# trioxane/consensus_clustering

Hardware: AMD Instinct MI355X
Metric: consensus fit wall-time + resample-clusterings/sec, n=50k d=128, 1/2/4/8 GPU (higher is better)
Workload: dtype f16x3 hi/lo, f32 accumulate (k-means MFMA) / i8 (co-association MFMA)

## Files before the change

consensus_clustering_amd/csrc/kmeans.hip:

```cpp
#include <hip/hip_runtime.h>

#include <algorithm>
#include <climits>
#include <cmath>
#include <cstdlib>
#include <cstdint>
#include <string>
#include <vector>

#include "kmeans_shared.hpp"

namespace {

using namespace cc::km;

constexpr int NT = 512;
constexpr int NW = 8;
constexpr int NDW = 4;
constexpr int NEW = NW - NDW;
constexpr int RT = 32;
constexpr int CW = 256;
constexpr int NLS = 8;
constexpr int NSS = 8;
constexpr int NLS_D = 3;
// ... 56 lines not shown
  const float* xnorm;
  int dreal;
  float scale, inv_scale, dscale, ndinv;
  const int32_t* idx;
  int m, h_begin, nh, T;
  const int32_t* units;
  int nU;
  int max_iter;
  double tol_rel;
  const double* kpp_u;
  int kpp_stride, n_init;
  const int32_t* kpp_pos;
  uint8_t* labels_out;
  int n, ldl, H;
  float* inertia_out;
  int32_t* niter_out;
  unsigned long long* stats;
  unsigned* counter;
  uint8_t* ws;
  size_t ws_per_wg, off_cen, off_cenn, off_cpos, off_dbuf, off_rdist, off_s64, off_c64, off_list;
  int Pws, Kws, Tws, seedmax;
  int lsm;
  int lseg;
};

__device__ int cc_km_dense_only = 0;
__device__ int cc_km_share_seed = 1;

struct State {
  int unit, P;
  float tol;
  int rr;
  unsigned seedfree;
  unsigned char K[PMAX], kidx[PMAX], init[PMAX], ntr[PMAX], st[PMAX], c[PMAX], cs[PMAX], sslot[PMAX];
  unsigned char need_sel[PMAX], to_run[PMAX], sbest[PMAX], lcur[PMAX];
  short cenoff[PMAX], pitem[PMAX];
  int iter[PMAX], amax[PMAX], nempty[PMAX];
  int pchg[PMAX];
  float pot32[PMAX], inert[PMAX];
  int cand[PMAX][TMAX];
  int nitems, ncols;
  unsigned char ikind[IMAX], iprob[IMAX], itr[IMAX];
  unsigned iw0[IMAX], iw1[IMAX];
  unsigned char lstep[NW][NLS], sstep[NW][NSS][2];
  unsigned char nlw[NW], nsw[NW];
  int4 sdesc[NW][NSS][2];
// ... 171 lines not shown
      const float t = x[d] - c[d];
      s = fmaf(t, t, s);
    }
    dist[r] = s;
    mymax = fmaxf(mymax, s);
  }
  for (int o = 32; o > 0; o >>= 1) mymax = fmaxf(mymax, __shfl_xor(mymax, o));
  if ((tid & 63) == 0) S.red_v[tid >> 6] = mymax;
  __syncthreads();
  double gmax = 0.0;
  for (int w = 0; w < NW; ++w) gmax = fmax(gmax, S.red_v[w]);
  if (tid == 0) {
    int ne = 0;
    for (int c = 0; c < K; ++c)
      if (S.cnt[off + c] == 0) S.map[ne++] = c;
    S.flag = ne;
  }
  __syncthreads();
  if (gmax == 0.0) return;
  relocate_farthest<NT, NW>(m, S.flag, S.map, dist, glab, a.X, idx, DP, off, Sm, S.cnt, S.red_v, S.red_i,
                            S.n_reloc, tid);
}

__device__ unsigned list_changes(const uint8_t* cur, const uint8_t* old, int m, int w, int lane, uint2* seg,
                                 unsigned cap) {
  const int rs = (((m + NW - 1) / NW) + 15) & ~15;
  const int r0 = w * rs, r1 = min(m, r0 + rs);
  unsigned n = 0;
  for (int b = r0; b < r1; b += 16 * 64) {
    const int r = b + 16 * lane;
    unsigned msk = 0;
    uint4 x = make_uint4(0, 0, 0, 0), y = x;
    if (r < r1) {
      x = *reinterpret_cast<const uint4*>(cur + r);
      y = *reinterpret_cast<const uint4*>(old + r);
      const unsigned xs[4] = {x.x, x.y, x.z, x.w}, ys[4] = {y.x, y.y, y.z, y.w};
#pragma unroll
      for (int q = 0; q < 4; ++q) {
        const unsigned dq = xs[q] ^ ys[q];
#pragma unroll
        for (int k = 0; k < 4; ++k) msk |= ((dq >> (8 * k)) & 0xFFu) ? (1u << (4 * q + k)) : 0u;
      }
    }
    const unsigned c = __popc(msk);
    unsigned pre = c;
#pragma unroll
    for (int o = 1; o < 64; o <<= 1) {
      const unsigned t = __shfl_up(pre, o);
      if (lane >= o) pre += t;
    }
    unsigned pos = n + pre - c;
    const unsigned xs[4] = {x.x, x.y, x.z, x.w}, ys[4] = {y.x, y.y, y.z, y.w};
    while (msk) {
      const int k = __builtin_ctz(msk);
      msk &= msk - 1;
      const unsigned nv = (xs[k >> 2] >> (8 * (k & 3))) & 0xFFu, ov = (ys[k >> 2] >> (8 * (k & 3))) & 0xFFu;
      if (pos < cap) seg[pos] = make_uint2(static_cast<unsigned>(r + k), ov | (nv << 8));
      ++pos;
    }
    n += __shfl(pre, 63);
  }
  return n;
}

template <int DP>
__device__ void apply_changes(const KArgs& a, const int32_t* idx, const uint2* lst, const unsigned* nseg,
                              bool full, const uint8_t* lab, float* acc, unsigned* cnt, int K, int lane) {
  constexpr int DL = DP >= 64 ? DP / 64 : 1;
  const bool dok = lane * DL < DP;
  const int d0 = dok ? lane * DL : 0;
  for (int e = lane; e < K * DP; e += 64) acc[e] = 0.f;
  if (lane < K) cnt[lane] = 0u;
  for (int sg = 0; sg < (full ? 1 : NW); ++sg) {
    const int n = full ? a.m : static_cast<int>(nseg[sg]);
    const uint2* ls = lst + static_cast<size_t>(sg) * a.lseg;
    for (int e0 = 0; e0 < n; e0 += 64) {
      const int e = e0 + lane;
      unsigned xr = 0, o = 0xFFu, nw = 0xFFu;
      if (e < n) {
        unsigned r;
        if (full) {
          r = static_cast<unsigned>(e);
          nw = lab[e];
// ... 39 lines not shown
                *reinterpret_cast<float2*>(q) = t;
              } else {
                *q += v[j][0];
              }
            }
            if (jo[j] < 0xFFu) {
              float* q = acc + jo[j] * DP + d0;
              if constexpr (DL == 2) {
                float2 t = *reinterpret_cast<float2*>(q);
                t.x -= v[j][0];
                t.y -= v[j][DL - 1];
                *reinterpret_cast<float2*>(q) = t;
              } else {
                *q -= v[j][0];
              }
            }
          }
        }
      }
    }
  }
}

typedef float v4f __attribute__((ext_vector_type(4)));
typedef float v2f __attribute__((ext_vector_type(2)));
typedef double v2d __attribute__((ext_vector_type(2)));
#define KM_GLOBAL __attribute__((address_space(1)))
#define KM_LDS __attribute__((address_space(3)))
template <class T>
__device__ __forceinline__ T* as_lds(T* p) {
  return (T*)(KM_LDS T*)p;
}

template <int DP>
struct SlotHalf {
  static constexpr int NQ = DP / 8;
  bool run = false;
  int p = 0, cl = 0, rot = 0;
  KM_LDS v4f* row = nullptr;
  template <class St>
  __device__ __forceinline__ SlotHalf(float* Sm, const St& S, int ncols) {
    const int tid = threadIdx.x, sl = tid >> 1;
    rot = tid / (128 / DP);
    row = (KM_LDS v4f*)(KM_LDS float*)Sm + (sl * DP + (tid & 1) * (DP / 2)) / 4;
    if (sl < ncols) {
      const int it = S.sitem[sl];
      if (it >= 0 && S.ikind[it] == IK_RUN) {
        run = true;
        p = S.iprob[it];
        cl = sl - S.ioff[it];
      }
    }
  }
  __device__ __forceinline__ int q(int j) const { return (j + rot) & (NQ - 1); }
};
// ... 64 lines not shown
      act[u] = true;
      rowu[u] = S.cenoff[S.iprob[it]] + (sl - S.ioff[it]);
      if (!(S.ichanged[it] & 2u)) {
        v[u] = s64[rowu[u] * (DP / 2) + lane];
        cu[u] = c64[rowu[u]];
      }
    }
#pragma unroll
    for (int u = 0; u < U; ++u) {
      if (!act[u]) continue;
      const int sl = s0 + u;
      const v2f f = Sm[sl * (DP / 2) + lane];
      const v2d t = {v[u].x + static_cast<double>(f.x), v[u].y + static_cast<double>(f.y)};
      s64[rowu[u] * (DP / 2) + lane] = t;
      Sm[sl * (DP / 2) + lane] = v2f{static_cast<float>(t.x), static_cast<float>(t.y)};
      if (lane == 0) {
        const int c = cu[u] + static_cast<int>(S.cnt[sl]);
        c64[rowu[u]] = c;
        S.cnt[sl] = static_cast<unsigned>(c);
      }
    }
  }
}
#undef KM_GLOBAL
#undef KM_LDS

template <class St>
__device__ void kpp_select(const KArgs& a, St& S, int p, const float* closest, int lane) {
  const int ntr = S.ntr[p];
  cc::km::kpp_select<RT, TMAX>(closest, a.m, a.T, kpp_uniforms(a.kpp_u, S.kidx[p], a.n_init, S.init[p], a.kpp_stride, S.c[p], ntr),
                               ntr, static_cast<double>(S.pot32[p]), S.cand[p], lane);
}

template <int NL, int NS>
struct EState {
  float iaccL[NL], iaccS[NS];
};
constexpr int FLUSH = 32;

__host__ __device__ constexpr int mstep_tile(int q) { return (q + 1) % NDW; }
static_assert(NEW == NDW, "one E/M wave per distance wave");

__device__ __forceinline__ int4 seed_desc(const KArgs& a, const State& S, int it, int T1) {
  if (it == 0xFF) return make_int4(0, CW, 0, CW);
  const unsigned w0 = S.iw0[it], w1 = S.iw1[it];
  const int slot = w1 & 31;
  const int dcf = iw_off(w0) | ((1 | ((iw_kind(w0) == IK_SEED) ? 2 : 0)) << 16);
  return make_int4((slot * T1 + ((w1 >> 8) & 7)) * a.lsm, dcf, (slot * T1 + ((w1 >> 11) & 7)) * a.lsm, dcf);
// ... 287 lines not shown
        }
      sacc0[dt] = mfma16(oh0, bh, sacc0[dt]);
      __builtin_amdgcn_sched_barrier(0);
#pragma unroll
      for (int k = 0; k < 4; ++k) rc[k] = rn[k];
    }
  }
}

template <int DP>
__device__ __forceinline__ void msum_out(const KArgs& a, State& S, float* Sm, const v16f (&sacc)[DP / 32],
                                         unsigned mcnt, int ct, int msl, int lr, int hh) {
#pragma unroll
  for (int dt = 0; dt < DP / 32; ++dt)
#pragma unroll
    for (int v = 0; v < 16; ++v) {
      const int s2 = 32 * ct + (v & 3) + 8 * (v >> 2) + 4 * hh;
      Sm[s2 * DP + 32 * dt + lr] = sacc[dt][v] * a.inv_scale;
    }
  const unsigned tot = mcnt + __shfl_xor(mcnt, 32);
  if (hh == 0) S.cnt[msl] = tot;
}

__device__ void schedule(const KArgs& a, State& S, const int32_t* idx, int dist_cost, bool sparse_ok) {
  const int P = S.P;
  for (int p = 0; p < P && S.seedfree; ++p) {
    if (S.st[p] != ST_WAIT) continue;
    const int s = __ffs(S.seedfree) - 1;
    S.seedfree &= ~(1u << s);
    S.sslot[p] = static_cast<unsigned char>(s);
    S.st[p] = ST_SEED;
    S.c[p] = 0;
  }
  int ni = 0, nc = 0, nls = 0, nss2 = 0;
  unsigned long long nseed = 0, nlloyd = 0, nm = 0;
  for (int p = 0; p < P; ++p) S.pitem[p] = -1;
  for (int p = 0; p < P; ++p) {
    if (S.st[p] != ST_SEED) continue;
    const int c = S.c[p];
    const int nt = (c == 0) ? 1 : S.ntr[p];
    if (nc + nt > CW || ni + nt > IMAX || nss2 + nt > 2 * (NEW * NSS + NDW * NSS_D)) continue;
    nss2 += nt;
    S.pitem[p] = static_cast<short>(ni);
    for (int t = 0; t < nt; ++t) {
      const int kind = (c == 0) ? IK_SEED0 : IK_SEED;
      S.ikind[ni] = static_cast<unsigned char>(kind);
      S.iprob[ni] = static_cast<unsigned char>(p);
// ... 91 lines not shown
    if (S.ikind[it] >= IK_RUN) continue;
    if (open_w >= 0) {
      S.sstep[open_w][S.nsw[open_w] - 1][1] = static_cast<unsigned char>(it);
      open_w = -1;
      continue;
    }
    int w = -1;
    for (int q = 0; q < NW; ++q)
      if (S.nsw[q] < (q < NDW ? NSS_D : NSS) && (w < 0 || wcost[q] < wcost[w])) w = q;
    S.sstep[w][S.nsw[w]++][0] = static_cast<unsigned char>(it);
    wcost[w] += KM_COST_SSTEP;
    open_w = w;
  }
  S.nitems = ni;
  S.ncols = nc;
  S.n_seed += nseed;
  S.n_lloyd += nlloyd;
  S.n_mrows += nm;
  if (ni > 0) {
    S.n_sweeps += 1;
    S.n_ctiles += static_cast<unsigned long long>((nc + 31) / 32) * a.T;
  }
}

template <int DP>
__global__ __launch_bounds__(NT, 1) void kmeans_kernel(KArgs a) {
  using LY = Lay<DP>;
  __shared__ __attribute__((aligned(16))) char smem[LY::TOTAL];
  char* ring = smem;
  float* Dt = reinterpret_cast<float*>(smem + LY::OFF_D);
  float* Sm = reinterpret_cast<float*>(smem);
  uint8_t* Ls = reinterpret_cast<uint8_t*>(smem + LY::OFF_LS);
  float* XN = reinterpret_cast<float*>(smem + LY::OFF_XN);
  State& S = *reinterpret_cast<State*>(smem + LY::OFF_ST);

  const int tid = threadIdx.x, lane = tid & 63;
  const int wave = __builtin_amdgcn_readfirstlane(tid >> 6);
  const int m = a.m, T = a.T;
  uint8_t* wsb = a.ws + static_cast<size_t>(blockIdx.x) * a.ws_per_wg;
  uint8_t* glab = wsb;
  double* s64 = reinterpret_cast<double*>(wsb + a.off_s64);
  int* c64 = reinterpret_cast<int*>(wsb + a.off_c64);
  uint2* clist = reinterpret_cast<uint2*>(wsb + a.off_list);
  float* cen = reinterpret_cast<float*>(wsb + a.off_cen);
  float* cenn = reinterpret_cast<float*>(wsb + a.off_cenn);
  int32_t* cpos = reinterpret_cast<int32_t*>(wsb + a.off_cpos);
  float* dbuf = reinterpret_cast<float*>(wsb + a.off_dbuf);
  float* rdist = reinterpret_cast<float*>(wsb + a.off_rdist);
  const int T1 = a.Tws + 1;
  if (tid == 0) S.n_lloyd = S.n_seed = S.n_mrows = S.n_reloc = S.n_sweeps = S.n_ctiles = S.n_sparse = S.n_changes = 0;

  for (;;) {
    __syncthreads();
    if (tid == 0) S.unit = static_cast<int>(atomicAdd(a.counter, 1u));
    __syncthreads();
    const int unit = S.unit;
    if (unit >= a.nh * a.nU) break;
    const int hb = unit / a.nU, g = unit - hb * a.nU;
    const int h = a.h_begin + hb;
    const int32_t* idx = a.idx + static_cast<size_t>(h) * m;
    const int32_t* gd = a.units + g * US;

    if (tid == 0) {
      const int P = gd[0];
      S.P = P;
      int o = 0;
      for (int p = 0; p < P; ++p) {
        S.K[p] = static_cast<unsigned char>(gd[1 + 4 * p]);
        S.kidx[p] = static_cast<unsigned char>(gd[2 + 4 * p]);
        S.init[p] = static_cast<unsigned char>(gd[3 + 4 * p]);
        S.ntr[p] = static_cast<unsigned char>(gd[4 + 4 * p]);
        S.st[p] = ST_WAIT;
        S.iter[p] = 0;
        S.pchg[p] = a.m;
        S.lcur[p] = 0;
        S.cenoff[p] = static_cast<short>(o);
        o += S.K[p];
        S.lead[p] = static_cast<unsigned char>(p);
        S.fgo[p] = 0;
      }
      if (cc_km_share_seed)
        for (int p = 0; p < P; ++p) {
          if (S.init[p] != 0) continue;
          int l = p;
          for (int q = 0; q < P; ++q)
            if (S.init[q] == 0 && S.ntr[q] == S.ntr[p] && (S.K[q] > S.K[l] || (S.K[q] == S.K[l] && q < l))) l = q;
          if (l != p) {
            S.lead[p] = static_cast<unsigned char>(l);
            S.st[p] = ST_FOLLOW;
          }
        }
      S.rr = 0;
      S.seedfree = (a.seedmax >= 32) ? 0xFFFFFFFFu : ((1u << a.seedmax) - 1u);
    }
    __syncthreads();
    const int P = S.P;
    for (size_t e = tid; e < static_cast<size_t>(2 * P) * a.lsm; e += NT) glab[e] = 0xFF;

    {
      double* red = reinterpret_cast<double*>(ring);
      double* mean = reinterpret_cast<double*>(ring) + NT;
      constexpr int NPH = NT / DP;
      const int d = tid % DP, ph = tid / DP;
      double s = 0.0;
      for (int r = ph; r < m; r += NPH) s += static_cast<double>(a.X[static_cast<size_t>(idx[r]) * DP + d]);
      red[ph * DP + d] = s;
      __syncthreads();
      if (tid < DP) {
        double t = 0.0;
        for (int k = 0; k < NPH; ++k) t += red[k * DP + tid];
        mean[tid] = t / m;
      }
      __syncthreads();
      const double mu = mean[d];
      double q = 0.0;
      for (int r = ph; r < m; r += NPH) {
        const double v = static_cast<double>(a.X[static_cast<size_t>(idx[r]) * DP + d]) - mu;
        q += v * v;
      }
      __syncthreads();
      red[ph * DP + d] = q;
      __syncthreads();
      if (tid == 0) {
        double tot = 0.0;
        for (int dd = 0; dd < a.dreal; ++dd) {
          double t = 0.0;
          for (int k = 0; k < NPH; ++k) t += red[k * DP + dd];
          tot += t / m;
        }
        S.tol = static_cast<float>(static_cast<float>(tot / a.dreal) * a.tol_rel);
      }
      __syncthreads();
    }

    for (;;) {
      KM_STAMP(swp);
      if (tid == 0) {
        if constexpr (kPair<DP>) {
          [[clang::always_inline]] schedule(a, S, idx, dist_cost<DP>(), kSparse<DP> && !cc_km_dense_only);
        } else {
          schedule(a, S, idx, dist_cost<DP>(), kSparse<DP> && !cc_km_dense_only);
        }
      }
      __syncthreads();
      const int nitems = S.nitems, ncols = S.ncols;
      if (nitems == 0) break;

      if (tid < ncols) {
        const int sr = S.srow[tid];
        S.cnorm[tid] = (sr >= 0) ? a.xnorm[sr] : (sr == INT_MIN ? __builtin_huge_valf() : cenn[-sr - 1]);
      }
      if (tid < 2 * RT * 4) Dt[(tid >> 2) * DSD + CW + (tid & 3)] = __builtin_huge_valf();
      if (tid < IMAX) S.iinert[tid] = 0.0;
      if (tid < NW * NSS * 2) {
        const int w = tid / (2 * NSS), i = (tid / 2) % NSS, h = tid & 1;
        S.sdesc[w][i][h] = seed_desc(a, S, S.sstep[w][i][h], T1);
      }
      const int hh = lane >> 5, lr = lane & 31;
      const bool pm = kPair<DP> && ncols <= 4 * 32;
      const int TP = (T + 1) >> 1;
#ifdef CC_KM_STAMPS
      unsigned long long st_acc[8] = {0, 0, 0, 0, 0, 0, 0, 0};
#endif
      if (wave < NDW) {
        const int nsub = __builtin_amdgcn_readfirstlane(static_cast<int>(32 * wave < ncols) +
                                                        static_cast<int>(32 * (wave + NDW) < ncols));
        h8 ah0[DP / 16], al0[DP / 16], ah1[DP / 16], al1[DP / 16];
// ... 235 lines not shown
        for (int k = 0; k < 7; ++k) atomicAdd(&a.stats[8 + 8 * wave + k], st_acc[k]);
#endif
      __syncthreads();

      KM_STAMP(pp0);
      if (tid < P) {
        const int p = tid;
        S.need_sel[p] = 0;
        S.to_run[p] = S.fgo[p];
        if (S.st[p] == ST_SEED && S.pitem[p] >= 0) {
          const int c = S.c[p];
          const KppDecision k = kpp_decide(S.iinert + S.pitem[p], S.ntr[p], c, S.cs[p]);
          S.pot32[p] = k.pot;
          S.cs[p] = static_cast<unsigned char>(k.cs);
          S.sbest[p] = static_cast<unsigned char>(k.best);
          cpos[p * a.Kws + c] = (c == 0) ? a.kpp_pos[S.kidx[p] * a.n_init + S.init[p]] : S.cand[p][k.best];
          S.c[p] = static_cast<unsigned char>(c + 1);
          if (c + 1 == S.K[p]) {
            S.to_run[p] = 1;
          } else {
            S.need_sel[p] = 1;
          }
        }
      }
      __syncthreads();
      if (tid == 0) {
        for (int p = 0; p < P; ++p)
          if (S.to_run[p]) {
            if (S.st[p] == ST_SEED) S.seedfree |= 1u << S.sslot[p];
            S.st[p] = ST_RUN;
            S.iter[p] = 0;
            S.pchg[p] = a.m;
          }
      }
      {
        int j = 0;
        for (int p = 0; p < P; ++p) {
          if (!S.need_sel[p]) continue;
          if ((j++ % NW) != wave) continue;
          const int ss = S.sslot[p];
          if constexpr (kPair<DP>) {
            [[clang::always_inline]] kpp_select(a, S, p, dbuf + (static_cast<size_t>(ss) * T1 + S.cs[p]) * a.lsm, lane);
          } else {
            kpp_select(a, S, p, dbuf + (static_cast<size_t>(ss) * T1 + S.cs[p]) * a.lsm, lane);
          }
        }
      }
      for (int p = 0; p < P; ++p) {
        if (!S.to_run[p]) continue;
        const int K = S.K[p], cp = S.lead[p] * a.Kws;
        for (int e = tid; e < K * DP; e += NT) {
          const int c = e / DP, d = e - c * DP;
          cen[(S.cenoff[p] + c) * DP + d] = a.X[static_cast<size_t>(idx[cpos[cp + c]]) * DP + d];
        }
        if (tid < K) cenn[S.cenoff[p] + tid] = row_sq(a.X + static_cast<size_t>(idx[cpos[cp + tid]]) * DP, a.dreal);
      }

// ... 18 lines not shown
            for (int w = 0; w < NW; ++w) {
              tot += S.lcnt[it][w];
              over |= S.lcnt[it][w] > static_cast<unsigned>(a.lseg);
            }
            S.pchg[S.iprob[it]] = static_cast<int>(tot);
            S.ichanged[it] = (tot != 0) | ((S.isparse[it] && over) ? 2u : 0u);
#ifdef CC_KM_STAMPS
            if (S.isparse[it] && over && a.stats) atomicAdd(&a.stats[117], 1ull);
#endif
          }
        }
      } else {
        if (tid < nitems) S.ichanged[tid] = 0;
        __syncthreads();
        for (int it = 0; it < nitems; ++it) {
          if (S.ikind[it] != IK_RUN) continue;
          const int p = S.iprob[it];
          if (labels_differ<NT>(glab + static_cast<size_t>(2 * p + 1 - S.lcur[p]) * a.lsm,
                                glab + static_cast<size_t>(2 * p + S.lcur[p]) * a.lsm, m, tid))
            S.ichanged[it] = 1;
        }
      }
      __syncthreads();
      if (tid == 0)
        for (int it = 0; it < nitems; ++it)
          if (S.ikind[it] >= IK_RUN) {
            S.lcur[S.iprob[it]] = static_cast<unsigned char>(1 - S.lcur[S.iprob[it]]);
            if (S.ikind[it] == IK_RUN) S.n_changes += static_cast<unsigned>(S.pchg[S.iprob[it]]);
          }
      __syncthreads();
      KM_STAMP(ppB);

      if constexpr (kSparse<DP>) {
        for (int e = tid; e < ncols * DP; e += NT) {
          const int sl = e / DP, d = e - sl * DP;
          const int it = S.sitem[sl];
          if (it < 0 || S.ikind[it] != IK_RUN || S.isparse[it] || sl - S.ioff[it] >= S.K[S.iprob[it]]) continue;
          const int row = S.cenoff[S.iprob[it]] + (sl - S.ioff[it]);
          s64[static_cast<size_t>(row) * DP + d] = static_cast<double>(Sm[e]);
          if (d == 0) c64[row] = static_cast<int>(S.cnt[sl]);
        }
        KM_STAMP(rs0);
        {
          int j = 0;
          for (int it = 0; it < nitems; ++it) {
            if (S.ikind[it] != IK_RUN || !S.isparse[it]) continue;
            if ((j++ % NW) != wave) continue;
            const int p = S.iprob[it], off = S.ioff[it];
            apply_changes<DP>(a, idx, clist + static_cast<size_t>(p) * NW * a.lseg, S.lcnt[it], (S.ichanged[it] & 2u) != 0,
                              glab + static_cast<size_t>(2 * p + S.lcur[p]) * a.lsm, Sm + static_cast<size_t>(off) * DP,
                              S.cnt + off, S.K[p], lane);
          }
        }
        KM_STAMP(rs1);
        __syncthreads();
        KM_STAMP(rs2);
        add_sparse_deltas<DP>(Sm, S, s64, c64, ncols);
        KM_STAMP(rs3);
        __syncthreads();
#ifdef CC_KM_STAMPS
        if (blockIdx.x == 0 && tid == 0 && a.stats) {
          atomicAdd(&a.stats[112], rs0 - ppB);
          atomicAdd(&a.stats[113], rs1 - rs0);
          atomicAdd(&a.stats[114], rs3 - rs2);
          atomicAdd(&a.stats[115], rs2 - rs1);
        }
#endif
      }

      KM_STAMP(ppC);
      if (tid == 0) {
        int f = 0;
        for (int it = 0; it < nitems; ++it) {
          if (S.ikind[it] != IK_RUN) continue;
          const int p = S.iprob[it], off = S.ioff[it];
          int ne = 0;
          for (int c = 0; c < S.K[p]; ++c) ne += (S.cnt[off + c] == 0);
          S.nempty[p] = ne;
          f |= (ne > 0);
        }
        S.flag = f;
      }
      __syncthreads();
      if (S.flag) {
        for (int it = 0; it < nitems; ++it) {
          if (S.ikind[it] != IK_RUN) continue;
          const int p = S.iprob[it];
          if (S.nempty[p] == 0) continue;
          if constexpr (kPair<DP>) {
            [[clang::always_inline]] relocate<DP>(a, idx, p, S.ioff[it], cen, Sm, S,
                                                  glab + static_cast<size_t>(2 * p + S.lcur[p]) * a.lsm, rdist, tid);
          } else {
            relocate<DP>(a, idx, p, S.ioff[it], cen, Sm, S, glab + static_cast<size_t>(2 * p + S.lcur[p]) * a.lsm,
                         rdist, tid);
          }
          __syncthreads();
        }
      }
      if (tid < nitems && S.ikind[tid] == IK_RUN) {
        const int p = S.iprob[tid], off = S.ioff[tid];
        int am = 0;
        for (int c = 1; c < S.K[p]; ++c)
          if (S.cnt[off + c] > S.cnt[off + am]) am = c;
        S.amax[p] = am;
      }
      __syncthreads();
// ... 29 lines not shown
                                        a.max_iter, S.iter[p]);
        S.st[p] = static_cast<unsigned char>(st);
        if (st == ST_DONE) S.inert[p] = static_cast<float>(S.iinert[it]);
      }
      __syncthreads();
      write_centres<DP>(Sm, S, cen, ncols);
      if (tid < ncols) {
        const int it = S.sitem[tid];
        if (it >= 0 && S.ikind[it] == IK_RUN) {
          const int p = S.iprob[it];
          if (S.st[p] != ST_DONE) cenn[S.cenoff[p] + (tid - S.ioff[it])] = row_sq(Sm + tid * DP, a.dreal);
        }
      }
      __syncthreads();
#ifdef CC_KM_STAMPS
      KM_STAMP(pp1);
      if (blockIdx.x == 0 && tid == 0 && a.stats) {
        atomicAdd(&a.stats[73], pp1 - pp0);
        atomicAdd(&a.stats[106], ppA - pp0);
        atomicAdd(&a.stats[107], ppB - ppA);
        atomicAdd(&a.stats[108], ppC - ppB);
        atomicAdd(&a.stats[109], pp1 - ppC);
        atomicAdd(&a.stats[116], cu1 - cu0);
      }
      if (tid == 0 && a.stats) {
        const int wv = (ncols + 31) / 32;
        atomicAdd(&a.stats[80 + wv], pp1 - swp);
        atomicAdd(&a.stats[96 + wv], 1ull);
        if (S.ikind[0] < IK_RUN) {
          atomicAdd(&a.stats[110], pp1 - swp);
          atomicAdd(&a.stats[111], 1ull);
        }
      }
#endif
    }

    for (int p0 = 0; p0 < P; p0 += a.n_init) {
      const auto lab = [&](int p) { return glab + static_cast<size_t>(2 * p + S.lcur[p]) * a.lsm; };
      const int best = best_of_inits<NT, KMAX>(p0, a.n_init, m, lab, [&](int p) { return S.inert[p]; }, S.map, S.flag, tid);
      write_fit<NT>(lab(best), idx, m, a.labels_out, a.n, a.ldl, S.kidx[p0], h, a.H, S.inert[best], S.iter[best],
                    a.inertia_out, a.niter_out, tid);
    }
  }
  if (tid == 0 && a.stats) {
    atomicAdd(&a.stats[0], S.n_lloyd);
    atomicAdd(&a.stats[1], S.n_seed);
    atomicAdd(&a.stats[2], S.n_mrows);
    atomicAdd(&a.stats[3], S.n_reloc);
    atomicAdd(&a.stats[4], S.n_sweeps);
    atomicAdd(&a.stats[5], S.n_ctiles);
    atomicAdd(&a.stats[6], S.n_sparse);
    atomicAdd(&a.stats[7], S.n_changes);
  }
}

__global__ void split_kernel(const float* X, long long total, int dpad, float scale, uint16_t* Xhl) {
  const long long i = static_cast<long long>(blockIdx.x) * blockDim.x + threadIdx.x;
  if (i >= total) return;
  const long long row = i / dpad;
  const int d = static_cast<int>(i - row * dpad);
  const float xs = X[i] * scale;
  const _Float16 hi = static_cast<_Float16>(xs);
  const _Float16 lo = static_cast<_Float16>(xs - static_cast<float>(hi));
  Xhl[row * 2 * dpad + d] = __builtin_bit_cast(uint16_t, hi);
  Xhl[row * 2 * dpad + dpad + d] = __builtin_bit_cast(uint16_t, lo);
}

struct WsLayout {
  int Pws = 0, Cws = 0, Kws = 0, Tws = 0, lseg = 0;
  size_t off_cen = 0, off_cenn = 0, off_cpos = 0, off_dbuf = 0, off_rdist = 0, off_s64 = 0, off_c64 = 0,
         off_list = 0, per_wg = 0;
};

int list_seg(int m) { return std::max(16, ((m / 16) + 15) & ~15); }

constexpr size_t WS_HEADER = 256;

WsLayout ws_layout(int m, int dpad, const int32_t* units, int nU, int seedmax) {
  WsLayout L;
  for (int g = 0; g < nU; ++g) {
    const int32_t* gd = units + static_cast<size_t>(g) * US;
    L.Pws = std::max(L.Pws, gd[0]);
    int cols = 0;
    for (int p = 0; p < gd[0]; ++p) {
      L.Kws = std::max(L.Kws, gd[1 + 4 * p]);
      L.Tws = std::max(L.Tws, gd[4 + 4 * p]);
      cols += gd[1 + 4 * p];
    }
    L.Cws = std::max(L.Cws, cols);
  }
  const auto al = align256;
  L.off_cen = al(static_cast<size_t>(2 * L.Pws) * ((m + 63) & ~63));
  L.off_cenn = L.off_cen + al(static_cast<size_t>(L.Cws) * dpad * sizeof(float));
  L.off_cpos = L.off_cenn + al(static_cast<size_t>(L.Cws) * sizeof(float));
  L.off_dbuf = L.off_cpos + al(static_cast<size_t>(L.Pws) * L.Kws * sizeof(int32_t));
  L.off_rdist = L.off_dbuf + al(static_cast<size_t>(seedmax) * (L.Tws + 1) * ((m + 63) & ~63) * sizeof(float));
  const bool sp = dpad == 128;
  L.off_s64 = L.off_rdist + al(static_cast<size_t>(m) * sizeof(float));
  L.off_c64 = L.off_s64 + (sp ? al(static_cast<size_t>(L.Cws) * dpad * sizeof(double)) : 0);
  L.off_list = L.off_c64 + (sp ? al(static_cast<size_t>(L.Cws) * sizeof(int)) : 0);
  L.lseg = list_seg(m);
  L.per_wg = L.off_list + (sp ? al(static_cast<size_t>(L.Pws) * NW * L.lseg * sizeof(uint2)) : 0);
  return L;
}

template <int DP>
void launch(const KArgs& a, unsigned blocks, hipStream_t st) {
  hipLaunchKernelGGL(kmeans_kernel<DP>, dim3(blocks), dim3(NT), 0, st, a);
}

}

extern "C" int cc_kmeans_plan(const int32_t* Ks, int nK, int n_init, int n_sub, int32_t* units,
                              int max_units) {
  if (!Ks || nK <= 0 || n_init <= 0 || n_sub <= 0 || !units || max_units <= 0) {
    cc::set_error("cc_kmeans_plan: bad arguments");
    return CC_ERR_ARG;
  }
  if (n_init > PMAX) {
    cc::set_error("cc_kmeans_plan: n_init must be <= 64");
    return CC_ERR_UNSUPPORTED;
  }
  std::vector<int> order(nK);
  for (int i = 0; i < nK; ++i) {
    if (Ks[i] < 1 || Ks[i] > KMAX) {
// ... 141 lines not shown
  a.kpp_u = kpp_u;
  a.kpp_stride = kpp_stride;
  a.n_init = n_init;
  a.kpp_pos = kpp_pos;
  a.labels_out = labels_nh;
  a.n = n;
  a.ldl = ldl;
  a.H = H;
  a.inertia_out = inertia;
  a.niter_out = n_iter;
  a.stats = stats;
  a.counter = static_cast<unsigned*>(workspace);
  a.ws = static_cast<uint8_t*>(workspace) + WS_HEADER;
  a.ws_per_wg = L.per_wg;
  a.off_cen = L.off_cen;
  a.off_cenn = L.off_cenn;
  a.off_cpos = L.off_cpos;
  a.off_dbuf = L.off_dbuf;
  a.off_rdist = L.off_rdist;
  a.off_s64 = L.off_s64;
  a.off_c64 = L.off_c64;
  a.off_list = L.off_list;
  a.lseg = L.lseg;
  a.Pws = L.Pws;
  a.Kws = L.Kws;
  a.Tws = L.Tws;
  a.seedmax = seedmax;
  a.lsm = (m + 63) & ~63;
  {
    static int dense_set = 0;
    const char* dm = std::getenv("CCMI_KM_DENSE");
    const int dense = (dm && dm[0] == '1') ? 1 : 0;
    if (dense != dense_set) {
      e = hipMemcpyToSymbolAsync(HIP_SYMBOL(cc_km_dense_only), &dense, sizeof(int), 0, hipMemcpyHostToDevice, st);
      if (e != hipSuccess) return hip_fail("cc_kmeans_batched", e);
      dense_set = dense;
    }
    static int share_set = 1;
    const char* sm = std::getenv("CCMI_KM_SHARE_SEED");
    const int share = (sm && sm[0] == '0') ? 0 : 1;
    if (share != share_set) {
      e = hipMemcpyToSymbolAsync(HIP_SYMBOL(cc_km_share_seed), &share, sizeof(int), 0, hipMemcpyHostToDevice, st);
      if (e != hipSuccess) return hip_fail("cc_kmeans_batched", e);
      share_set = share;
    }
    if (const char* ls = std::getenv("CCMI_KM_LSEG")) {
// ... 13 lines not shown
```

Measured before the change: 11330.

## Parallelize k-means scheduler across a wave and unroll serial per-sweep loops

Result: faster. 11850, median of 6 (+4.6%).

```diff
diff --git a/consensus_clustering_amd/csrc/kmeans.hip b/consensus_clustering_amd/csrc/kmeans.hip
--- a/consensus_clustering_amd/csrc/kmeans.hip
+++ b/consensus_clustering_amd/csrc/kmeans.hip
@@ -102,6 +102,9 @@
   int Pws, Kws, Tws, seedmax;
   int lsm;
   int lseg;
+#ifdef CC_KM_SCHED_CHECK
+  size_t off_chk;
+#endif
 };
 
 __device__ int cc_km_dense_only = 0;
@@ -319,43 +322,83 @@
                             S.n_reloc, tid);
 }
 
-__device__ unsigned list_changes(const uint8_t* cur, const uint8_t* old, int m, int w, int lane, uint2* seg,
-                                 unsigned cap) {
+typedef float v4f __attribute__((ext_vector_type(4)));
+typedef float v2f __attribute__((ext_vector_type(2)));
+typedef double v2d __attribute__((ext_vector_type(2)));
+typedef unsigned v4u __attribute__((ext_vector_type(4)));
+typedef unsigned v2u __attribute__((ext_vector_type(2)));
+#define KM_GLOBAL __attribute__((address_space(1)))
+#define KM_LDS __attribute__((address_space(3)))
+template <class T>
+__device__ __forceinline__ T* as_lds(T* p) {
+  return (T*)(KM_LDS T*)p;
+}
+template <class T>
+__device__ __forceinline__ KM_GLOBAL T* as_global(T* p) {
+  return (KM_GLOBAL T*)reinterpret_cast<uintptr_t>(p);
+}
+
+#ifndef KM_CMP_NB
+#define KM_CMP_NB 6
+#endif
+__device__ __noinline__ unsigned list_changes(const uint8_t* cur_, const uint8_t* old_, int m, int w, int lane,
+                                              uint2* seg_, unsigned cap) {
+  const KM_GLOBAL uint8_t* cur = as_global(cur_);
+  const KM_GLOBAL uint8_t* old = as_global(old_);
+  KM_GLOBAL v2u* seg = (KM_GLOBAL v2u*)reinterpret_cast<uintptr_t>(seg_);
+  constexpr int NB = KM_CMP_NB, BR = 16 * 64;
   const int rs = (((m + NW - 1) / NW) + 15) & ~15;
   const int r0 = w * rs, r1 = min(m, r0 + rs);
-  unsigned n = 0;
-  for (int b = r0; b < r1; b += 16 * 64) {
-    const int r = b + 16 * lane;
-    unsigned msk = 0;
-    uint4 x = make_uint4(0, 0, 0, 0), y = x;
-    if (r < r1) {
-      x = *reinterpret_cast<const uint4*>(cur + r);
-      y = *reinterpret_cast<const uint4*>(old + r);
-      const unsigned xs[4] = {x.x, x.y, x.z, x.w}, ys[4] = {y.x, y.y, y.z, y.w};
+  unsigned n = 0, cl = 0;
+  for (int b0 = r0; b0 < r1; b0 += NB * BR) {
+    v4u x[NB], y[NB];
+#pragma unroll
+    for (int u = 0; u < NB; ++u) {
+      const int r = b0 + u * BR + 16 * lane;
+      x[u] = y[u] = v4u{0u, 0u, 0u, 0u};
+      if (r < r1) {
+        x[u] = *reinterpret_cast<const KM_GLOBAL v4u*>(cur + r);
+        y[u] = *reinterpret_cast<const KM_GLOBAL v4u*>(old + r);
+      }
+    }
+#pragma unroll
+    for (int u = 0; u < NB; ++u) {
+      if (b0 + u * BR >= r1) break;
+      const int r = b0 + u * BR + 16 * lane;
+      unsigned msk = 0;
 #pragma unroll
       for (int q = 0; q < 4; ++q) {
-        const unsigned dq = xs[q] ^ ys[q];
+        const unsigned dq = x[u][q] ^ y[u][q];
 #pragma unroll
         for (int k = 0; k < 4; ++k) msk |= ((dq >> (8 * k)) & 0xFFu) ? (1u << (4 * q + k)) : 0u;
       }
-    }
-    const unsigned c = __popc(msk);
-    unsigned pre = c;
-#pragma unroll
-    for (int o = 1; o < 64; o <<= 1) {
-      const unsigned t = __shfl_up(pre, o);
-      if (lane >= o) pre += t;
-    }
-    unsigned pos = n + pre - c;
-    const unsigned xs[4] = {x.x, x.y, x.z, x.w}, ys[4] = {y.x, y.y, y.z, y.w};
-    while (msk) {
-      const int k = __builtin_ctz(msk);
-      msk &= msk - 1;
-      const unsigned nv = (xs[k >> 2] >> (8 * (k & 3))) & 0xFFu, ov = (ys[k >> 2] >> (8 * (k & 3))) & 0xFFu;
-      if (pos < cap) seg[pos] = make_uint2(static_cast<unsigned>(r + k), ov | (nv << 8));
-      ++pos;
-    }
-    n += __shfl(pre, 63);
+      const unsigned c = __popc(msk);
+      if (cap == 0u) {
+        cl += c;
+        continue;
+      }
+      if (__ballot(msk != 0u) == 0ull) continue;
+      unsigned pre = c;
+#pragma unroll
+      for (int o = 1; o < 64; o <<= 1) {
+        const unsigned t = __shfl_up(pre, o);
+        if (lane >= o) pre += t;
+      }
+      unsigned pos = n + pre - c;
+      while (msk) {
+        const int k = __builtin_ctz(msk);
+        msk &= msk - 1;
+        const unsigned nv = (x[u][k >> 2] >> (8 * (k & 3))) & 0xFFu, ov = (y[u][k >> 2] >> (8 * (k & 3))) & 0xFFu;
+        if (pos < cap) seg[pos] = v2u{static_cast<unsigned>(r + k), ov | (nv << 8)};
+        ++pos;
+      }
+      n += __shfl(pre, 63);
+    }
+  }
+  if (cap == 0u) {
+#pragma unroll
+    for (int o = 32; o > 0; o >>= 1) cl += __shfl_xor(cl, o);
+    n = cl;
   }
   return n;
 }
@@ -441,15 +484,6 @@
   }
 }
 
-typedef float v4f __attribute__((ext_vector_type(4)));
-typedef float v2f __attribute__((ext_vector_type(2)));
-typedef double v2d __attribute__((ext_vector_type(2)));
-#define KM_GLOBAL __attribute__((address_space(1)))
-#define KM_LDS __attribute__((address_space(3)))
-template <class T>
-__device__ __forceinline__ T* as_lds(T* p) {
-  return (T*)(KM_LDS T*)p;
-}
 
 template <int DP>
 struct SlotHalf {
@@ -560,8 +594,6 @@
     }
   }
 }
-#undef KM_GLOBAL
-#undef KM_LDS
 
 template <class St>
 __device__ void kpp_select(const KArgs& a, St& S, int p, const float* closest, int lane) {
@@ -895,7 +927,8 @@
   if (hh == 0) S.cnt[msl] = tot;
 }
 
-__device__ void schedule(const KArgs& a, State& S, const int32_t* idx, int dist_cost, bool sparse_ok) {
+#ifdef CC_KM_SCHED_CHECK
+__device__ __noinline__ void schedule(const KArgs& a, State& S, const int32_t* idx, int dist_cost, bool sparse_ok) {
   const int P = S.P;
   for (int p = 0; p < P && S.seedfree; ++p) {
     if (S.st[p] != ST_WAIT) continue;
@@ -1033,6 +1066,259 @@
     S.n_ctiles += static_cast<unsigned long long>((nc + 31) / 32) * a.T;
   }
 }
+#endif
+
+#ifndef KM_TOL_U
+#define KM_TOL_U 16
+#endif
+template <int DP, bool SQ>
+__device__ __noinline__ double tol_pass(const float* X_, const int32_t* idx_, int m, double mu) {
+  const KM_GLOBAL float* X = as_global(X_);
+  const KM_GLOBAL int32_t* idx = as_global(idx_);
+  constexpr int NPH = NT / DP, U = KM_TOL_U;
+  const int d = threadIdx.x % DP, ph = threadIdx.x / DP;
+  const auto add = [&](double s, float x) {
+    if constexpr (SQ) {
+      const double v = static_cast<double>(x) - mu;
+      return __builtin_fma(v, v, s);
+    } else {
+      return s + static_cast<double>(x);
+    }
+  };
+  double s = 0.0;
+  int r = ph;
+  for (; r + (U - 1) * NPH < m; r += U * NPH) {
+    int ix[U];
+    float x[U];
+#pragma unroll
+    for (int u = 0; u < U; ++u) ix[u] = idx[r + u * NPH];
+#pragma unroll
+    for (int u = 0; u < U; ++u) x[u] = X[static_cast<size_t>(ix[u]) * DP + d];
+#pragma unroll
+    for (int u = 0; u < U; ++u) s = add(s, x[u]);
+  }
+  for (; r < m; r += NPH) s = add(s, X[static_cast<size_t>(idx[r]) * DP + d]);
+  return s;
+}
+
+__device__ __forceinline__ int lpt_wave(const int (&wcost)[NW], const int (&nst)[NW], int cap_d, int cap_e) {
+  int w = -1, best = 0;
+#pragma unroll
+  for (int q = 0; q < NW; ++q)
+    if (nst[q] < (q < NDW ? cap_d : cap_e) && (w < 0 || wcost[q] < best)) {
+      w = q;
+      best = wcost[q];
+    }
+  return w;
+}
+
+__device__ void schedule_wave(State& S_, const int32_t* idx_, const int32_t* kpp_pos_, int n_init, int m, int T,
+                              int dist_cost, bool sparse_ok, int lane) {
+  State& S = *as_lds(&S_);
+  const KM_GLOBAL int32_t* idx = as_global(idx_);
+  const KM_GLOBAL int32_t* kpp_pos = as_global(kpp_pos_);
+  const int P = __builtin_amdgcn_readfirstlane(S.P);
+  const bool in = lane < P;
+  int st = in ? S.st[lane] : 0xFF;
+  int c = in ? S.c[lane] : 0;
+  const int K = in ? S.K[lane] : 0, ntr = in ? S.ntr[lane] : 0;
+  const int lead = in ? S.lead[lane] : 0;
+  const int pchg = in ? S.pchg[lane] : 0;
+  {
+    unsigned seedfree = __builtin_amdgcn_readfirstlane(S.seedfree);
+    unsigned long long wait = __ballot(st == ST_WAIT);
+    int s_new = -1;
+    while (wait && seedfree) {
+      const int p = __builtin_ctzll(wait), s = __builtin_ctz(seedfree);
+      wait &= wait - 1;
+      seedfree &= seedfree - 1;
+      if (lane == p) s_new = s;
+    }
+    if (s_new >= 0) {
+      st = ST_SEED;
+      c = 0;
+      S.sslot[lane] = static_cast<unsigned char>(s_new);
+      S.st[lane] = ST_SEED;
+      S.c[lane] = 0;
+    }
+    if (lane == 0) S.seedfree = seedfree;
+  }
+  int ni = 0, nc = 0, nss2 = 0;
+  int myit = -1;
+  const int ntv = (c == 0) ? 1 : ntr;
+  for (unsigned long long sm = __ballot(st == ST_SEED); sm; sm &= sm - 1) {
+    const int p = __builtin_ctzll(sm);
+    const int nt = __builtin_amdgcn_readlane(ntv, p);
+    if (nc + nt > CW || ni + nt > IMAX || nss2 + nt > 2 * (NEW * NSS + NDW * NSS_D)) continue;
+    nss2 += nt;
+    if (lane == p) myit = ni;
+    ni += nt;
+    nc += nt;
+  }
+  const int nis = ni;
+  if (st == ST_SEED && myit >= 0) {
+    const int kind = (c == 0) ? IK_SEED0 : IK_SEED;
+    const int cs = (kind == IK_SEED0) ? 0 : S.cs[lane];
+    const unsigned sslot = S.sslot[lane];
+    for (int t = 0; t < ntv; ++t) {
+      const int it = myit + t;
+      S.ikind[it] = static_cast<unsigned char>(kind);
+      S.iprob[it] = static_cast<unsigned char>(lane);
+      S.ioff[it] = static_cast<short>(it);
+      S.incol[it] = 1;
+      S.itr[it] = static_cast<unsigned char>(t);
+      const int wslot = (kind == IK_SEED0) ? 0 : ((t < cs) ? t : t + 1);
+      S.iw0[it] = (static_cast<unsigned>(kind) << 24) | (static_cast<unsigned>(lane) << 16) | (1u << 8) |
+                  static_cast<unsigned>(it);
+      S.iw1[it] = (static_cast<unsigned>(wslot) << 11) | (static_cast<unsigned>(cs) << 8) |
+                  (static_cast<unsigned>(t) << 5) | sslot;
+      const int pos = (c == 0) ? kpp_pos[S.kidx[lane] * n_init + S.init[lane]] : S.cand[lane][t];
+      S.sitem[it] = static_cast<short>(it);
+      S.scl[it] = -1;
+      S.srow[it] = idx[pos];
+    }
+  }
+  {
+    const int stl = __shfl(st, lead), itl = __shfl(myit, lead), cl = __shfl(c, lead);
+    if (in) S.fgo[lane] = static_cast<unsigned char>(st == ST_FOLLOW && stl == ST_SEED && itl >= 0 && cl + 1 == K);
+  }
+  const bool lrun = st == ST_RUN || st == ST_FINAL;
+  const int sparse = (sparse_ok && st == ST_RUN && pchg <= m / 8) ? 1 : 0;
+  const int K4 = (K + 3) & ~3;
+  int nls = 0, first_skip = -1, last = -1, nrun = 0, nsp = 0, klloyd = 0;
+  int myoff = 0, itK = 0;
+  const int rr = __builtin_amdgcn_readfirstlane(S.rr);
+  {
+    const unsigned long long rm = __ballot(lrun), below = rr ? (~0ull >> (64 - rr)) : 0ull;
+#pragma unroll 1
+    for (int half = 0; half < 2; ++half)
+      for (unsigned long long q = half ? (rm & below) : (rm & ~below); q; q &= q - 1) {
+        const int p = __builtin_ctzll(q);
+        const int Kp = __builtin_amdgcn_readlane(K, p), K4p = __builtin_amdgcn_readlane(K4, p);
+        const int off = (nc + 3) & ~3;
+        if (off + K4p > CW || ni + 1 > IMAX || nls + 1 > NEW * NLS + NDW * NLS_D) {
+          if (first_skip < 0) first_skip = p;
+          continue;
+        }
+        if (lane == p) {
+          myit = ni;
+          myoff = off;
+        }
+        if (lane == nls) itK = Kp;
+        ++ni;
+        ++nls;
+        nc = off + K4p;
+        last = p;
+        klloyd += Kp;
+        nrun += __builtin_amdgcn_readlane(static_cast<int>(st == ST_RUN), p);
+        nsp += __builtin_amdgcn_readlane(sparse, p);
+      }
+  }
+  const bool litem = lrun && myit >= nis;
+  if (litem) {
+    if (myit == nis)
+      for (int s = nis; s < myoff; ++s) {
+        S.sitem[s] = -1;
+        S.scl[s] = -1;
+        S.srow[s] = INT_MIN;
+      }
+    const int kind = (st == ST_RUN) ? IK_RUN : IK_FINAL;
+    S.isparse[myit] = static_cast<unsigned char>(sparse);
+    S.ikind[myit] = static_cast<unsigned char>(kind);
+    S.iprob[myit] = static_cast<unsigned char>(lane);
+    S.ioff[myit] = static_cast<short>(myoff);
+    S.incol[myit] = static_cast<short>(K);
+    S.itr[myit] = 0;
+    S.iw0[myit] = (static_cast<unsigned>(1 - S.lcur[lane]) << 30) | (static_cast<unsigned>(kind) << 24) |
+                  (static_cast<unsigned>(lane) << 16) | (static_cast<unsigned>(K) << 8) | static_cast<unsigned>(myoff);
+    S.iw1[myit] = 0;
+    const int cenoff = S.cenoff[lane];
+    const bool msl = st == ST_RUN && !sparse;
+    for (int s = 0; s < K4; ++s) {
+      S.sitem[myoff + s] = static_cast<short>(s < K ? myit : -1);
+      S.scl[myoff + s] = static_cast<short>((msl && s < K) ? s : -1);
+      S.srow[myoff + s] = (s < K) ? -(cenoff + s) - 1 : INT_MIN;
+    }
+  }
+  if (in) S.pitem[lane] = static_cast<short>(myit);
+  int wcost[NW], nlw[NW], nsw[NW];
+  {
+    const bool dense = litem && st == ST_RUN && !sparse;
+    unsigned mt = 0;
+#pragma unroll
+    for (int j = 0; j < CW / 32; ++j)
+      if (__ballot(dense && (myoff >> 5) <= j && j <= ((myoff + K - 1) >> 5)) != 0ull) mt |= 1u << j;
+#pragma unroll
+    for (int w = 0; w < NW; ++w) {
+      wcost[w] = 0;
+      nlw[w] = nsw[w] = 0;
+      if (w < NDW) {
+#pragma unroll
+        for (int j = w; j < CW / 32; j += NDW) wcost[w] += (32 * j < nc) ? dist_cost : 0;
+      } else {
+#pragma unroll
+        for (int j = mstep_tile(w - NDW); j < CW / 32; j += NEW) wcost[w] += ((mt >> j) & 1u) ? KM_COST_MSTEP : 0;
+      }
+    }
+  }
+  static_assert(NW * NLS == 64 && NW * NSS * 2 == 128, "the step tables are reset a lane each");
+  (&S.lstep[0][0])[lane] = 0xFF;
+  (&S.sstep[0][0][0])[2 * lane] = 0xFF;
+  (&S.sstep[0][0][0])[2 * lane + 1] = 0xFF;
+  for (int i = 0; i < nls; ++i) {
+    const int Ki = __builtin_amdgcn_readlane(itK, i);
+    const int w = lpt_wave(wcost, nlw, NLS_D, NLS);
+    int n = 0;
+#pragma unroll
+    for (int q = 0; q < NW; ++q)
+      if (q == w) {
+        n = nlw[q]++;
+        wcost[q] += (Ki + 7) / 8 * KM_COST_LCHUNK + KM_COST_LBASE;
+      }
+    if (lane == 0) S.lstep[w][n] = static_cast<unsigned char>(nis + i);
+  }
+  for (int it = 0; it < nis; it += 2) {
+    const int w = lpt_wave(wcost, nsw, NSS_D, NSS);
+    int n = 0;
+#pragma unroll
+    for (int q = 0; q < NW; ++q)
+      if (q == w) {
+        n = nsw[q]++;
+        wcost[q] += KM_COST_SSTEP;
+      }
+    if (lane == 0) {
+      S.sstep[w][n][0] = static_cast<unsigned char>(it);
+      if (it + 1 < nis) S.sstep[w][n][1] = static_cast<unsigned char>(it + 1);
+    }
+  }
+  {
+    int ln = 0, sn = 0;
+#pragma unroll
+    for (int q = 0; q < NW; ++q) {
+      ln = (lane == q) ? nlw[q] : ln;
+      sn = (lane == q) ? nsw[q] : sn;
+    }
+    if (lane < NW) {
+      S.nlw[lane] = static_cast<unsigned char>(ln);
+      S.nsw[lane] = static_cast<unsigned char>(sn);
+    }
+  }
+  if (lane == 0) {
+    S.rr = (first_skip >= 0) ? first_skip : (last >= 0 ? (last + 1) % P : rr);
+    S.nitems = ni;
+    S.ncols = nc;
+    S.n_seed += static_cast<unsigned long long>(nis) * m;
+    S.n_lloyd += static_cast<unsigned long long>(klloyd) * m;
+    S.n_mrows += static_cast<unsigned long long>(nrun) * m;
+    S.n_sparse += static_cast<unsigned>(nsp);
+    if (ni > 0) {
+      S.n_sweeps += 1;
+      S.n_ctiles += static_cast<unsigned long long>((nc + 31) / 32) * T;
+    }
+  }
+}
+#undef KM_GLOBAL
+#undef KM_LDS
 
 template <int DP>
 __global__ __launch_bounds__(NT, 1) void kmeans_kernel(KArgs a) {
@@ -1071,6 +1357,7 @@
     const int h = a.h_begin + hb;
     const int32_t* idx = a.idx + static_cast<size_t>(h) * m;
     const int32_t* gd = a.units + g * US;
+    KM_STAMP(us0);
 
     if (tid == 0) {
       const int P = gd[0];
@@ -1106,16 +1393,16 @@
     }
     __syncthreads();
     const int P = S.P;
+    KM_STAMP(us1);
     for (size_t e = tid; e < static_cast<size_t>(2 * P) * a.lsm; e += NT) glab[e] = 0xFF;
+    KM_STAMP(us2);
 
     {
       double* red = reinterpret_cast<double*>(ring);
       double* mean = reinterpret_cast<double*>(ring) + NT;
       constexpr int NPH = NT / DP;
       const int d = tid % DP, ph = tid / DP;
-      double s = 0.0;
-      for (int r = ph; r < m; r += NPH) s += static_cast<double>(a.X[static_cast<size_t>(idx[r]) * DP + d]);
-      red[ph * DP + d] = s;
+      red[ph * DP + d] = tol_pass<DP, false>(a.X, idx, m, 0.0);
       __syncthreads();
       if (tid < DP) {
         double t = 0.0;
@@ -1123,12 +1410,7 @@
         mean[tid] = t / m;
       }
       __syncthreads();
-      const double mu = mean[d];
-      double q = 0.0;
-      for (int r = ph; r < m; r += NPH) {
-        const double v = static_cast<double>(a.X[static_cast<size_t>(idx[r]) * DP + d]) - mu;
-        q += v * v;
-      }
+      const double q = tol_pass<DP, true>(a.X, idx, m, mean[d]);
       __syncthreads();
       red[ph * DP + d] = q;
       __syncthreads();
@@ -1143,17 +1425,42 @@
       }
       __syncthreads();
     }
+    KM_STAMP(us3);
 
     for (;;) {
       KM_STAMP(swp);
-      if (tid == 0) {
+#ifdef CC_KM_SCHED_CHECK
+      for (unsigned e = tid; e < sizeof(State) / 4; e += NT)
+        reinterpret_cast<unsigned*>(wsb + a.off_chk)[e] = reinterpret_cast<const unsigned*>(&S)[e];
+      __syncthreads();
+#endif
+      if (wave == 0) {
+#ifdef KM_SCHED_INLINE
         if constexpr (kPair<DP>) {
-          [[clang::always_inline]] schedule(a, S, idx, dist_cost<DP>(), kSparse<DP> && !cc_km_dense_only);
-        } else {
-          schedule(a, S, idx, dist_cost<DP>(), kSparse<DP> && !cc_km_dense_only);
-        }
-      }
+          [[clang::always_inline]] schedule_wave(S, idx, a.kpp_pos, a.n_init, m, T, dist_cost<DP>(),
+                                                 kSparse<DP> && !cc_km_dense_only, lane);
+        } else
+#endif
+        {
+          [[clang::noinline]] schedule_wave(S, idx, a.kpp_pos, a.n_init, m, T, dist_cost<DP>(),
+                                            kSparse<DP> && !cc_km_dense_only, lane);
+        }
+      }
+      KM_STAMP(sch1);
       __syncthreads();
+#ifdef CC_KM_SCHED_CHECK
+      {
+        State& R = *reinterpret_cast<State*>(wsb + a.off_chk);
+        if (tid == 0) schedule(a, R, idx, dist_cost<DP>(), kSparse<DP> && !cc_km_dense_only);
+        __syncthreads();
+        unsigned bad = 0;
+        for (unsigned e = tid; e < sizeof(State) / 4; e += NT)
+          bad += reinterpret_cast<const unsigned*>(&R)[e] != reinterpret_cast<const unsigned*>(&S)[e];
+        if (bad && a.stats) atomicAdd(&a.stats[122], static_cast<unsigned long long>(bad));
+        if (tid == 0 && a.stats && S.nitems > 0) atomicAdd(&a.stats[123], 1ull);
+        __syncthreads();
+      }
+#endif
       const int nitems = S.nitems, ncols = S.ncols;
       if (nitems == 0) break;
 
@@ -1435,17 +1742,15 @@
             S.need_sel[p] = 1;
           }
         }
+        if (S.to_run[p]) {
+          if (S.st[p] == ST_SEED)
+            __hip_atomic_fetch_or(&S.seedfree, 1u << S.sslot[p], __ATOMIC_RELAXED, __HIP_MEMORY_SCOPE_WORKGROUP);
+          S.st[p] = ST_RUN;
+          S.iter[p] = 0;
+          S.pchg[p] = a.m;
+        }
       }
       __syncthreads();
-      if (tid == 0) {
-        for (int p = 0; p < P; ++p)
-          if (S.to_run[p]) {
-            if (S.st[p] == ST_SEED) S.seedfree |= 1u << S.sslot[p];
-            S.st[p] = ST_RUN;
-            S.iter[p] = 0;
-            S.pchg[p] = a.m;
-          }
-      }
       {
         int j = 0;
         for (int p = 0; p < P; ++p) {
@@ -1510,12 +1815,15 @@
         }
       }
       __syncthreads();
-      if (tid == 0)
-        for (int it = 0; it < nitems; ++it)
-          if (S.ikind[it] >= IK_RUN) {
-            S.lcur[S.iprob[it]] = static_cast<unsigned char>(1 - S.lcur[S.iprob[it]]);
-            if (S.ikind[it] == IK_RUN) S.n_changes += static_cast<unsigned>(S.pchg[S.iprob[it]]);
-          }
+      KM_STAMP(fl0);
+      if (tid == 0) S.flag = 0;
+      if (tid < nitems && S.ikind[tid] >= IK_RUN) {
+        const int p = S.iprob[tid];
+        S.lcur[p] = static_cast<unsigned char>(1 - S.lcur[p]);
+        if (S.ikind[tid] == IK_RUN)
+          __hip_atomic_fetch_add(&S.n_changes, static_cast<unsigned long long>(static_cast<unsigned>(S.pchg[p])),
+                                 __ATOMIC_RELAXED, __HIP_MEMORY_SCOPE_WORKGROUP);
+      }
       __syncthreads();
       KM_STAMP(ppB);
 
@@ -1557,19 +1865,15 @@
       }
 
       KM_STAMP(ppC);
-      if (tid == 0) {
-        int f = 0;
-        for (int it = 0; it < nitems; ++it) {
-          if (S.ikind[it] != IK_RUN) continue;
-          const int p = S.iprob[it], off = S.ioff[it];
-          int ne = 0;
-          for (int c = 0; c < S.K[p]; ++c) ne += (S.cnt[off + c] == 0);
-          S.nempty[p] = ne;
-          f |= (ne > 0);
-        }
-        S.flag = f;
+      if (tid < nitems && S.ikind[tid] == IK_RUN) {
+        const int p = S.iprob[tid], off = S.ioff[tid];
+        int ne = 0;
+        for (int c = 0; c < S.K[p]; ++c) ne += (S.cnt[off + c] == 0);
+        S.nempty[p] = ne;
+        if (ne > 0) S.flag = 1;
       }
       __syncthreads();
+      KM_STAMP(ec1);
       if (S.flag) {
         for (int it = 0; it < nitems; ++it) {
           if (S.ikind[it] != IK_RUN) continue;
@@ -1645,6 +1949,8 @@
         atomicAdd(&a.stats[108], ppC - ppB);
         atomicAdd(&a.stats[109], pp1 - ppC);
         atomicAdd(&a.stats[116], cu1 - cu0);
+        atomicAdd(&a.stats[118], sch1 - swp);
+        atomicAdd(&a.stats[121], (ec1 - ppC) + (ppB - fl0));
       }
       if (tid == 0 && a.stats) {
         const int wv = (ncols + 31) / 32;
@@ -1658,12 +1964,22 @@
 #endif
     }
 
+    KM_STAMP(out0);
     for (int p0 = 0; p0 < P; p0 += a.n_init) {
       const auto lab = [&](int p) { return glab + static_cast<size_t>(2 * p + S.lcur[p]) * a.lsm; };
       const int best = best_of_inits<NT, KMAX>(p0, a.n_init, m, lab, [&](int p) { return S.inert[p]; }, S.map, S.flag, tid);
       write_fit<NT>(lab(best), idx, m, a.labels_out, a.n, a.ldl, S.kidx[p0], h, a.H, S.inert[best], S.iter[best],
                     a.inertia_out, a.niter_out, tid);
     }
+#ifdef CC_KM_STAMPS
+    KM_STAMP(out1);
+    if (blockIdx.x == 0 && tid == 0 && a.stats) {
+      atomicAdd(&a.stats[74], us3 - us0);
+      atomicAdd(&a.stats[119], us3 - us2);
+      atomicAdd(&a.stats[120], us2 - us1);
+      atomicAdd(&a.stats[75], out1 - out0);
+    }
+#endif
   }
   if (tid == 0 && a.stats) {
     atomicAdd(&a.stats[0], S.n_lloyd);
@@ -1692,7 +2008,7 @@
 struct WsLayout {
   int Pws = 0, Cws = 0, Kws = 0, Tws = 0, lseg = 0;
   size_t off_cen = 0, off_cenn = 0, off_cpos = 0, off_dbuf = 0, off_rdist = 0, off_s64 = 0, off_c64 = 0,
-         off_list = 0, per_wg = 0;
+         off_list = 0, off_chk = 0, per_wg = 0;
 };
 
 int list_seg(int m) { return std::max(16, ((m / 16) + 15) & ~15); }
@@ -1723,7 +2039,11 @@
   L.off_c64 = L.off_s64 + (sp ? al(static_cast<size_t>(L.Cws) * dpad * sizeof(double)) : 0);
   L.off_list = L.off_c64 + (sp ? al(static_cast<size_t>(L.Cws) * sizeof(int)) : 0);
   L.lseg = list_seg(m);
-  L.per_wg = L.off_list + (sp ? al(static_cast<size_t>(L.Pws) * NW * L.lseg * sizeof(uint2)) : 0);
+  L.off_chk = L.off_list + (sp ? al(static_cast<size_t>(L.Pws) * NW * L.lseg * sizeof(uint2)) : 0);
+  L.per_wg = L.off_chk;
+#ifdef CC_KM_SCHED_CHECK
+  L.per_wg += al(sizeof(State));
+#endif
   return L;
 }
 
@@ -1911,6 +2231,9 @@
   a.off_c64 = L.off_c64;
   a.off_list = L.off_list;
   a.lseg = L.lseg;
+#ifdef CC_KM_SCHED_CHECK
+  a.off_chk = L.off_chk;
+#endif
   a.Pws = L.Pws;
   a.Kws = L.Kws;
   a.Tws = L.Tws;
```
